# ClashLuke/LocAtE

Measured on AMD Instinct MI355X. Metric: images/sec (G+D step) 64x64 bs=64, higher is better.
Workload: dtype f32 (contractions fp32-faithful on the matrix cores: 2 x scaled fp16 operand pieces / 3 MFMAs per slice where the operand's largest magnitude comes with it, else 3 x bf16 pieces / 6 MFMAs; fp32 accumulate); 1 GPU; LocAtE G+D step, 64x64 RGB, batch 64 per GPU (the fp32 variant - the reference's own precision - of BASELINE.json configs[1]: 64x64 RGB bs 64), self/feature attention at 16x16 and 64x64, random-init weights; global_batch=64, image_size=64, parallelism=dp1, launch=hipGraph replay, G-step generator pass on a second stream

## Files before the change

### locate_amd/csrc/conv.hip

```cpp
#include "igemm.h"



struct PackBatch {
    PackArgs ph[4];
};

__device__ __forceinline__ void pack_tables(const PackArgs& a, int k) {
    int* koff = reinterpret_cast<int*>(a.out + (size_t)a.rows * a.ld);
    unsigned char* ktap = reinterpret_cast<unsigned char*>(koff + a.rows);
    const int T = a.TH * a.TW;
    int off = 0, tap = 31;
    if (k < a.K && T > 0) {
        const int c = k / T, t = k - c * T;
        const int th = t / a.TW, tw = t - th * a.TW;
        off = 4 * (c * a.gHW + (a.dy0 + a.dys * th) * a.gW + a.dx0 + a.dxs * tw - a.dmin);
        tap = t;
    }
    koff[k] = off;
    ktap[k] = (unsigned char)tap;
}

__device__ __forceinline__ void pack_publish_absmax(float m, const PackArgs* phases, int nphase, float* red) {
    m = wave_max(m);
// ... 504 lines not shown
    int nsteps = total_steps - step0;
    if (nsteps > per_split) nsteps = per_split;
    if (nsteps < 0) nsteps = 0;

    const float4* aptr[A_PT];
    bool a_ok[A_PT];
    int a_row[A_PT], a_c4[A_PT];
#pragma unroll
    for (int i = 0; i < A_PT; ++i) {
        const int idx = tid + i * 256;
        const int idc = ((i + 1) * 256 <= A_F4 || idx < A_F4) ? idx : 0;
        a_row[i] = idc / (BM / 4);
        a_c4[i] = idc - a_row[i] * (BM / 4);
        const int col = m0 + a_c4[i] * 4;
        a_ok[i] = col < ph.ld;
        aptr[i] = reinterpret_cast<const float4*>(ph.wp + (long long)(step0 * BK + a_row[i]) * ph.ld + (a_ok[i] ? col : 0));
    }
    const long long a_step = (long long)BK * ph.ld / 4;
    int kidx = step0 * BK + kgrp * KPT;

    float breg[KPT];
    float4 areg[A_PT];
    auto issue_loads = [&]() {
#pragma unroll
        for (int i = 0; i < A_PT; ++i) {
            areg[i] = *aptr[i];
            aptr[i] += a_step;
        }
        const int ks = __builtin_amdgcn_readfirstlane(kidx);
        const i32x8 offs = *reinterpret_cast<const i32x8*>(ph.koff + ks);
        const unsigned long long taps = *reinterpret_cast<const unsigned long long*>(ph.ktap + ks);
#pragma unroll
        for (int j = 0; j < KPT; ++j) breg[j] = gather_load(gc, offs[j], (unsigned)(taps >> (8 * j)) & 31u);
        kidx += BK;
    };
    auto store_tiles = [&](int buf) {
#pragma unroll
        for (int i = 0; i < A_PT; ++i) {
            const int idx = tid + i * 256;
            if ((i + 1) * 256 <= A_F4 || idx < A_F4) {
                float4 v = areg[i];
                v.x = a_ok[i] ? v.x : 0.f; v.y = a_ok[i] ? v.y : 0.f; v.z = a_ok[i] ? v.z : 0.f; v.w = a_ok[i] ? v.w : 0.f;
                *reinterpret_cast<float4*>(&As[buf][a_row[i]][a_c4[i] * 4]) = v;
            }
        }
#pragma unroll
        for (int j = 0; j < KPT; ++j) Bs[buf][kgrp * KPT + j][ncol] = breg[j];
    };

    if (nsteps > 0) {
        issue_loads();
        store_tiles(0);
    }
    __syncthreads();
    const int lrow = lane >> 5, lcol = lane & 31;
    for (int s = 0; s < nsteps; ++s) {
        const int buf = s & 1;
        issue_loads();
        __builtin_amdgcn_sched_barrier(0);
#pragma unroll
        for (int k2 = 0; k2 < BK / 2; ++k2) {
            float a[TM], b[TN];
#pragma unroll
            for (int i = 0; i < TM; ++i) a[i] = As[buf][k2 * 2 + lrow][(wm * TM + i) * 32 + lcol];
#pragma unroll
            for (int j = 0; j < TN; ++j) b[j] = Bs[buf][k2 * 2 + lrow][(wn * TN + j) * 32 + lcol];
#pragma unroll
            for (int i = 0; i < TM; ++i)
#pragma unroll
                for (int j = 0; j < TN; ++j) acc[i][j] = __builtin_amdgcn_mfma_f32_32x32x2f32(a[i], b[j], acc[i][j], 0, 0, 0);
        }
        __builtin_amdgcn_sched_barrier(0);
        store_tiles(buf ^ 1);
        __syncthreads();
    }

    igemm_epilogue<WGM, WGN, TM, TN>(p, ph, acc, col_scale, N, n0, m0, zsplit, wm, wn, lane, nullptr, p.ksplit > 1);
}

#define B6_BK 16

#define IG_FOUR_BLOCKS_TILES 3
#define IG_FOUR_BLOCKS_MIN 2
template <int WGM, int WGN, int TM, int TN, int NP, int NW = 4>
__global__ void __launch_bounds__(64 * NW, (NW == 8 ? 1 : (WGM * TM > 4 ? 2 : ((WGM * TM * TN <= IG_FOUR_BLOCKS_TILES && WGM * TM * TN >= IG_FOUR_BLOCKS_MIN && NP <= 2) ? 4 : 3)))) conv_igemm_bx6_kernel(const IgParams p) {
    constexpr int BK = 4 * NW, KB = BK / 8, KS = BK / 16, NT = 64 * NW;
    constexpr int BM = WGM * TM * 32;
    constexpr int BN = WGN * TN * 32;
    static_assert(NW == 4 || NW == 8, "four or eight waves");
    static_assert(WGM * WGN == NW, "wave grid");
    static_assert(BN == 128 && KB * BN == NT, "one gathered fragment (k-block) per thread and stage");
    static_assert(KB * BM <= 2 * NT, "at most two weight fragments per thread and stage");
    static_assert(B6_BK == 16, "the host's split-K accounting counts 16-deep steps");
    constexpr bool A2 = KB * BM > NT;
    static_assert(2 * BK <= IG_TAIL && (IG_TAIL % 8) == 0, "panel tail shorter than the prefetch distance");

    constexpr int A_U4 = 2 * NP * KB * BM, B_U4 = 2 * NP * KB * BN;
    constexpr int EPI_U4 = (NW * 32 * 33 + 8 + 3) / 4;
    constexpr int SMEM_U4 = A_U4 + B_U4 > EPI_U4 ? A_U4 + B_U4 : EPI_U4;
    __shared__ uint4 smem[SMEM_U4];
    uint4 (*As)[NP][KB][BM] = reinterpret_cast<uint4 (*)[NP][KB][BM]>(smem);
    uint4 (*Bs)[NP][KB][BN] = reinterpret_cast<uint4 (*)[NP][KB][BN]>(smem + A_U4);

    int bx, by, bz;
    xcd_tile(bx, by, bz, p.tile_nphase);
    const int zphase = bz / p.ksplit, zsplit = bz - zphase * p.ksplit;
    const IgPhase& ph = p.ph[zphase];
    const int N = p.B * ph.QH * ph.QW;
    const int n0 = bx * BN;
    const int m0 = by * BM;
    if (n0 >= N) return;

    const int tid = threadIdx.x, lane = tid & 63, wid = tid >> 6;
    const int wm = wid / WGN, wn = wid % WGN;

    const int ncol = tid % BN;
    const int kgrp = __builtin_amdgcn_readfirstlane(tid / BN);
    const GatherCol gc = gather_setup(p, ph, n0 + ncol, N);
    float col_scale[TN];
    igemm_col_scales<WGM, WGN, TM, TN>(p, ph, col_scale, N, n0, wn, lane);
    float b_scale = 1.0f, a_unscale = 1.0f, b_unscale = 1.0f;
    if constexpr (NP == 2) {
        const int kb_ = f16_scale_exp(absmax_read(p.b_absmax));
        const int ka_ = f16_scale_exp(__builtin_amdgcn_readfirstlane(*ph.a_absmax));
        b_scale = pow2f(kb_);
        a_unscale = pow2f(-ka_);
        b_unscale = pow2f(-kb_);
    }

    f32x16 acc[TM][TN];
#pragma unroll
    for (int i = 0; i < TM; ++i)
#pragma unroll
        for (int j = 0; j < TN; ++j)
#pragma unroll
            for (int r = 0; r < 16; ++r) acc[i][j][r] = 0.0f;

    const int total_steps = ph.Kpad / BK;
    const int per_split = (total_steps + p.ksplit - 1) / p.ksplit;
    const int step0 = zsplit * per_split;
    int nsteps = total_steps - step0;
    if (nsteps > per_split) nsteps = per_split;
    if (nsteps < 0) nsteps = 0;

    const bool a_thread = KB * BM == NT || tid < KB * BM;
    const int a_kb = a_thread ? tid / BM : 0, a_m = a_thread ? tid % BM : 0;
    const uint4* ap = ph.w3 + (long long)(step0 * KB + a_kb) * ph.ld + (m0 + a_m);
    const long long a_step = (long long)KB * ph.ld, a_plane = ph.w3_plane;
    const bool b_thread = A2 && tid + NT < KB * BM;
    const int b_kb = b_thread ? (tid + NT) / BM : 0, b_m = b_thread ? (tid + NT) % BM : 0;
    const uint4* bp = ph.w3 + (long long)(step0 * KB + b_kb) * ph.ld + (m0 + b_m);
    int kidx = step0 * BK + kgrp * 8;

    uint4 areg0, areg1, areg2;
    uint4 areg3, areg4, areg5;
    float breg[8];
    i32x8 offs = *reinterpret_cast<const i32x8*>(ph.koff + __builtin_amdgcn_readfirstlane(kidx));
    unsigned long long taps = *reinterpret_cast<const unsigned long long*>(ph.ktap + __builtin_amdgcn_readfirstlane(kidx));
    auto issue_loads = [&]() {
        areg0 = ap[0];
        if constexpr (NP >= 2) areg1 = ap[a_plane];
        if constexpr (NP == 3) areg2 = ap[2 * a_plane];
        ap += a_step;
        if constexpr (A2) {
            areg3 = bp[0];
            if constexpr (NP >= 2) areg4 = bp[a_plane];
            if constexpr (NP == 3) areg5 = bp[2 * a_plane];
            bp += a_step;
        }
#pragma unroll
        for (int j = 0; j < 8; ++j) breg[j] = gather_load(gc, offs[j], (unsigned)(taps >> (8 * j)) & 31u);
        kidx += BK;
        const int ks = __builtin_amdgcn_readfirstlane(kidx);
        offs = *reinterpret_cast<const i32x8*>(ph.koff + ks);
        taps = *reinterpret_cast<const unsigned long long*>(ph.ktap + ks);
    };
    auto store_tiles = [&](int buf) {
        if (a_thread) {
            As[buf][0][a_kb][a_m] = areg0;
            if constexpr (NP >= 2) As[buf][NP >= 2 ? 1 : 0][a_kb][a_m] = areg1;
            if constexpr (NP == 3) As[buf][NP - 1][a_kb][a_m] = areg2;
        }
        if constexpr (A2) {
            if (b_thread) {
                As[buf][0][b_kb][b_m] = areg3;
                if constexpr (NP >= 2) As[buf][NP >= 2 ? 1 : 0][b_kb][b_m] = areg4;
                if constexpr (NP == 3) As[buf][NP - 1][b_kb][b_m] = areg5;
            }
        }
        if constexpr (NP == 2) {
            uint4 h, l;
            float v[8];
#pragma unroll
            for (int j = 0; j < 8; ++j) v[j] = breg[j];
            split2_f16x8(v, b_scale, h, l);
            Bs[buf][0][kgrp][ncol] = h;
            Bs[buf][NP - 1][kgrp][ncol] = l;
        } else if constexpr (NP == 3) {
            uint4 h, m, l;
            float v[8];
#pragma unroll
            for (int j = 0; j < 8; ++j) v[j] = breg[j];
            split3_trunc_x8(v, h, m, l);
            Bs[buf][0][kgrp][ncol] = h;
            Bs[buf][NP - 2][kgrp][ncol] = m;
            Bs[buf][NP - 1][kgrp][ncol] = l;
        } else {
            bf16x8 h;
#pragma unroll
            for (int j = 0; j < 8; ++j) h[j] = (__bf16)breg[j];
            Bs[buf][0][kgrp][ncol] = *reinterpret_cast<uint4*>(&h);
        }
    };

    if (nsteps > 0) {
        issue_loads();
        store_tiles(0);
        issue_loads();
    }
    __syncthreads();
    const int lrow = lane >> 5, lcol = lane & 31;
    constexpr int PROD = NP == 3 ? 6 : (NP == 2 ? 3 : 1);
    constexpr int NMF = TM * TN * PROD, HALF = KS == 1 ? NMF / 2 : NMF;
    using frag_t = typename std::conditional<NP == 2, f16x8, bf16x8>::type;
    for (int s = 0; s < nsteps; ++s) {
        const int buf = s & 1;
        frag_t a[TM][NP], b[TN][NP];
        auto fragments = [&](int ksub) {
#pragma unroll
            for (int i = 0; i < TM; ++i)
#pragma unroll
                for (int q = 0; q < NP; ++q) a[i][q] = *reinterpret_cast<const frag_t*>(&As[buf][q][2 * ksub + lrow][(wm * TM + i) * 32 + lcol]);
#pragma unroll
            for (int j = 0; j < TN; ++j)
#pragma unroll
                for (int q = 0; q < NP; ++q) b[j][q] = *reinterpret_cast<const frag_t*>(&Bs[buf][q][2 * ksub + lrow][(wn * TN + j) * 32 + lcol]);
        };
        fragments(0);
        auto mfmas = [&](int lo, int hi) {
#pragma unroll
            for (int i = 0; i < TM; ++i)
#pragma unroll
                for (int j = 0; j < TN; ++j) {
                    const int base = (i * TN + j) * PROD;
                    if constexpr (NP == 2) {
                        if (base + 0 >= lo && base + 0 < hi) acc[i][j] = __builtin_amdgcn_mfma_f32_32x32x16_f16(a[i][1], b[j][0], acc[i][j], 0, 0, 0);
                        if (base + 1 >= lo && base + 1 < hi) acc[i][j] = __builtin_amdgcn_mfma_f32_32x32x16_f16(a[i][0], b[j][1], acc[i][j], 0, 0, 0);
                        if (base + 2 >= lo && base + 2 < hi) acc[i][j] = __builtin_amdgcn_mfma_f32_32x32x16_f16(a[i][0], b[j][0], acc[i][j], 0, 0, 0);
                    } else if constexpr (NP == 3) {
                        if (base + 0 >= lo && base + 0 < hi) acc[i][j] = __builtin_amdgcn_mfma_f32_32x32x16_bf16(a[i][NP - 1], b[j][0], acc[i][j], 0, 0, 0);
                        if (base + 1 >= lo && base + 1 < hi) acc[i][j] = __builtin_amdgcn_mfma_f32_32x32x16_bf16(a[i][0], b[j][NP - 1], acc[i][j], 0, 0, 0);
                        if (base + 2 >= lo && base + 2 < hi) acc[i][j] = __builtin_amdgcn_mfma_f32_32x32x16_bf16(a[i][NP - 2], b[j][NP - 2], acc[i][j], 0, 0, 0);
                        if (base + 3 >= lo && base + 3 < hi) acc[i][j] = __builtin_amdgcn_mfma_f32_32x32x16_bf16(a[i][NP - 2], b[j][0], acc[i][j], 0, 0, 0);
                        if (base + 4 >= lo && base + 4 < hi) acc[i][j] = __builtin_amdgcn_mfma_f32_32x32x16_bf16(a[i][0], b[j][NP - 2], acc[i][j], 0, 0, 0);
                        if (base + 5 >= lo && base + 5 < hi) acc[i][j] = __builtin_amdgcn_mfma_f32_32x32x16_bf16(a[i][0], b[j][0], acc[i][j], 0, 0, 0);
                    } else {
                        if (base >= lo && base < hi) acc[i][j] = __builtin_amdgcn_mfma_f32_32x32x16_bf16(a[i][0], b[j][0], acc[i][j], 0, 0, 0);
                    }
                }
        };
        __builtin_amdgcn_sched_barrier(0);
        mfmas(0, HALF);
        __builtin_amdgcn_sched_barrier(0);
        store_tiles(buf ^ 1);
        __builtin_amdgcn_sched_barrier(0);
        issue_loads();
        if constexpr (KS == 1) {
            mfmas(HALF, NMF);
        } else {
            fragments(1);
            mfmas(0, NMF);
        }
        if constexpr (NP >= 2) {
#pragma unroll
            for (int k = 0; k < (KS == 1 ? NMF - HALF : NMF); ++k) {
                __builtin_amdgcn_sched_group_barrier(0x008, 1, 0);
                __builtin_amdgcn_sched_group_barrier(0x020, 1, 0);
                __builtin_amdgcn_sched_group_barrier(0x002, 3, 0);
            }
        }
        __syncthreads();
    }
    if constexpr (NP == 2) {
#pragma unroll
        for (int i = 0; i < TM; ++i)
#pragma unroll
            for (int j = 0; j < TN; ++j)
#pragma unroll
                for (int r = 0; r < 16; ++r) acc[i][j][r] = (acc[i][j][r] * a_unscale) * b_unscale;
    }
    float* const stage = reinterpret_cast<float*>(smem) + wid * (32 * 33);
    bool combined = false;
    if (p.ksplit > 1 && p.combine) {
        constexpr int FR = TM * TN * 4;
        const int tile = (zphase * (int)gridDim.y + by) * (int)gridDim.x + bx;
        const int ntiles = p.nphase * (int)gridDim.y * (int)gridDim.x;
        const unsigned tile_bytes = FR * NT * 16;
        __amdgpu_buffer_rsrc_t srs = __builtin_amdgcn_make_buffer_rsrc(p.slab, 0, (int)((unsigned)p.ksplit * ntiles * tile_bytes), 0x00020000);
        const unsigned my = ((unsigned)(zsplit * ntiles + tile)) * tile_bytes + (unsigned)tid * 16u;
#pragma unroll
        for (int i = 0; i < TM; ++i)
#pragma unroll
            for (int j = 0; j < TN; ++j)
#pragma unroll
                for (int q = 0; q < 4; ++q) {
                    u32x4 v;
                    v[0] = __float_as_uint(acc[i][j][4 * q + 0]); v[1] = __float_as_uint(acc[i][j][4 * q + 1]);
                    v[2] = __float_as_uint(acc[i][j][4 * q + 2]); v[3] = __float_as_uint(acc[i][j][4 * q + 3]);
                    __builtin_amdgcn_raw_buffer_store_b128(v, srs, (int)(my + (unsigned)(((i * TN + j) * 4 + q) * NT * 16)), 0, 16);
                }
        asm volatile("s_waitcnt vmcnt(0)" ::: "memory");
        __syncthreads();
        unsigned* const flag = reinterpret_cast<unsigned*>(smem) + NW * 32 * 33 + 4;
        if (tid == 0) {
            const unsigned ticket = __hip_atomic_fetch_add(p.counters + tile, 1u, __ATOMIC_RELAXED, __HIP_MEMORY_SCOPE_AGENT);
            const bool last = ticket == (unsigned)(p.ksplit - 1);
            if (last) {
                __hip_atomic_store(p.counters + tile, 0u, __ATOMIC_RELAXED, __HIP_MEMORY_SCOPE_AGENT);
                __builtin_amdgcn_fence(__ATOMIC_ACQUIRE, "agent");
                asm volatile("s_waitcnt vmcnt(0)" ::: "memory");
            }
            *flag = last ? 1u : 0u;
        }
        __syncthreads();
        if (*flag == 0u) return;
        const unsigned t0 = (unsigned)tile * tile_bytes + (unsigned)tid * 16u;
        const unsigned zstride = (unsigned)ntiles * tile_bytes;
#pragma unroll
        for (int i = 0; i < TM; ++i)
#pragma unroll
            for (int j = 0; j < TN; ++j)
#pragma unroll
                for (int r = 0; r < 16; ++r) acc[i][j][r] = 0.0f;
        constexpr int HB = 4, ZB = 4;
#pragma unroll
        for (int h0 = 0; h0 < FR; h0 += HB) {
            for (int z0 = 0; z0 < p.ksplit; z0 += ZB) {
                u32x4 v[ZB][HB];
#pragma unroll
                for (int zz = 0; zz < ZB; ++zz)
#pragma unroll
                    for (int f = 0; f < HB; ++f)
                        v[zz][f] = __builtin_amdgcn_raw_buffer_load_b128(srs, (int)(t0 + (unsigned)(z0 + zz) * zstride + (unsigned)((h0 + f) * NT * 16)), 0, 16);
#pragma unroll
                for (int zz = 0; zz < ZB; ++zz)
#pragma unroll
                    for (int f = 0; f < HB; ++f) {
                        const int g = h0 + f, i = g / (TN * 4), j = (g / 4) % TN, q = g % 4;
#pragma unroll
                        for (int e = 0; e < 4; ++e) acc[i][j][4 * q + e] += __uint_as_float(v[zz][f][e]);
                    }
            }
        }
        __syncthreads();
        combined = true;
    }
    igemm_epilogue<WGM, WGN, TM, TN>(p, ph, acc, col_scale, N, n0, m0, combined ? 0 : zsplit, wm, wn, lane, stage, p.ksplit > 1 && !combined);
}

__global__ void __launch_bounds__(256) igemm_slab_reduce_kernel(const float* __restrict__ slab, float* __restrict__ out,
                                                                const float* __restrict__ bias, const float* __restrict__ scale,
                                                                int scale_bg, int scale_stride, int B, int M, int plane,
                                                                long long out_bs, long long slab_stride, int ksplit,
// ... 220 lines not shown
template <int PX>
static void launch_pointwise_px(const IgParams& p, hipStream_t st) {
    const long long npx = (long long)p.B * p.H * p.W / PX;
    const int blocks = (int)((npx + 255) / 256);
    const int mt = (p.M + 15) / 16;
    if (mt == 1) conv_pointwise_kernel<16, PX><<<blocks, 256, 0, st>>>(p);
    else if (mt == 2) conv_pointwise_kernel<32, PX><<<blocks, 256, 0, st>>>(p);
    else if (mt == 3) conv_pointwise_kernel<48, PX><<<blocks, 256, 0, st>>>(p);
    else conv_pointwise_kernel<64, PX><<<blocks, 256, 0, st>>>(p);
}

static void launch_pointwise(const IgParams& p, hipStream_t st) {
    if ((long long)p.B * p.H * p.W >= (long long)knob_int("LOCATE_PX2_MIN", 2 * 256 * 1024)) launch_pointwise_px<2>(p, st);
    else launch_pointwise_px<1>(p, st);
}

static int pick_bm(int M);
static int igemm_bm(int M, int nmax, int nphase) {
    if (M % 192 == 0 && M >= 192 && !path_disabled("tall") && !path_disabled("bx6")) {
        const long long tiles = (long long)((nmax + 127) / 128) * (M / 192) * nphase;
        if (tiles >= 512) return 192;
    }
    return pick_bm(M);
}

static int pick_bm(int M) {
    const int cands[4] = {128, 96, 64, 32};
    int best = 128, best_pad = 1 << 30;
    for (int i = 0; i < 4; ++i) {
        const int pad = round_up(M, cands[i]);
        if (pad < best_pad) { best_pad = pad; best = cands[i]; }
    }
    return best;
}

static int igemm_ksplit(int M, int nmax, int nphase, int min_kpad) {
    const int bm = igemm_bm(M, nmax, nphase);
    const long long tiles = (long long)((nmax + 127) / 128) * ((M + bm - 1) / bm) * nphase;
    const int slots = bm == 192 ? 512 : 768;
    if (tiles >= slots || (tiles >= 512 && tiles % 256 == 0)) return 1;
    const int steps = min_kpad / IG_BK;
    long long want = (slots + tiles - 1) / tiles;
    const int min_steps = (long long)M * nmax <= (1 << 16) ? 2 : 8;
    if (steps < 8) return 1;
    const int max_split = steps / min_steps > 0 ? steps / min_steps : 1;
    if (want > max_split) want = max_split;
    if (want > 64) want = 64;
    if (want > knob_int("LOCATE_KS_MAX", 64)) want = knob_int("LOCATE_KS_MAX", 64);
    return want < 1 ? 1 : (int)want;
}

#define IG_MAX_COUNTERS 1024
struct SplitPlan {
    int ksplit, combine, gx, gy;
    size_t slab_floats;
};

static SplitPlan igemm_split_plan(const IgParams& p, int nmax, bool have_counters) {
    SplitPlan sp;
    const int bm = igemm_bm(p.M, nmax, p.nphase);
    int min_kpad = 1 << 30;
    for (int i = 0; i < p.nphase; ++i) min_kpad = p.ph[i].Kpad < min_kpad ? p.ph[i].Kpad : min_kpad;
    int ks = igemm_ksplit(p.M, nmax, p.nphase, min_kpad);
    if (ks > min_kpad / IG_BK) ks = min_kpad / IG_BK;
    if (ks < 1) ks = 1;
    sp.ksplit = ks;
    sp.gx = (nmax + 127) / 128;
    sp.gy = (p.M + bm - 1) / bm;
    const long long ntiles = (long long)sp.gx * sp.gy * p.nphase;
    const long long tile_floats = (long long)bm * 128;
    const long long legacy = ks > 1 ? (long long)ks * p.B * p.M * p.OH * p.OW : 0;
    const long long fused = ks > 1 ? (long long)ks * ntiles * tile_floats : 0;
    sp.combine = have_counters && ks > 1 && (long long)ks * tile_floats * 4 <= (512 << 10) && ntiles <= IG_MAX_COUNTERS &&
                 fused * 4 < (1ll << 31) && (p.precision == 1 || !path_disabled("bx6")) && !path_disabled("combine");
    sp.slab_floats = (size_t)(sp.combine ? fused : legacy);
    return sp;
}

void launch_slab_reduce(const IgParams& p, hipStream_t st) {
    igemm_slab_reduce_kernel<<<stream_grid(p.slab_stride, 256), 256, 0, st>>>(p.slab, p.out, p.bias, p.scale, p.scale_bg, p.scale_stride, p.B, p.M, p.OH * p.OW,
                                                                              p.out_bs, p.slab_stride, p.ksplit, p.act_out, p.act_bs, p.mul_pre, p.mul_bs, p.out_absmax);
}

static int launch_igemm(IgParams& p, int nmax, void* slab_ws, unsigned* counters, hipStream_t st, const char* who) {
    p.tile_nphase = (path_disabled("phasefast") || (long long)p.OH * p.OW < 1024) ? 1 : p.nphase;
    if (p.win) return launch_win_igemm(p, nmax, slab_ws, counters, st, who);
    if (skinny_ok(p)) {
        p.ksplit = 1;
        launch_skinny(p, st);
        LOCATE_LAUNCH_CHECK(who);
        return LOCATE_OK;
    }
    if (pointwise_ok(p)) {
        p.ksplit = 1;
        launch_pointwise(p, st);
        LOCATE_LAUNCH_CHECK(who);
        return LOCATE_OK;
    }
    const int bm = igemm_bm(p.M, nmax, p.nphase);
    const SplitPlan sp = igemm_split_plan(p, nmax, counters != nullptr);
    p.ksplit = sp.ksplit;
    p.combine = sp.combine;
    p.counters = counters;
    p.slab = static_cast<float*>(slab_ws);
    p.slab_stride = (long long)p.B * p.M * p.OH * p.OW;
    dim3 grid(sp.gx, sp.gy, p.nphase * p.ksplit);
    for (int i = 0; i < p.nphase; ++i)
        LOCATE_REQUIRE(round_up(p.M, bm) <= p.ph[i].ld, "%s: tile height %d does not divide the panel width %d", who, bm, p.ph[i].ld);
    if (p.precision == 3) {
        launch_fp8_igemm(p, grid, bm, st);
        LOCATE_LAUNCH_CHECK(who);
        if (p.ksplit > 1 && !p.combine) {
            LOCATE_REQUIRE(p.slab_stride < (1ll << 31), "%s: split-K output of %lld elements exceeds the 32-bit index range", who, p.slab_stride);
            launch_slab_reduce(p, st);
            LOCATE_LAUNCH_CHECK(who);
        }
        return LOCATE_OK;
    }
    const bool w8 = !path_disabled("w8") && !path_disabled("bx6") && (bm == 128 || bm == 64) &&
                    (long long)grid.x * grid.y * grid.z <= knob_int("LOCATE_W8_MAX", 320);
    if (p.precision == 2) LOCATE_REQUIRE(!path_disabled("bx6"), "%s: fp16 pieces need the bf16/fp16 MFMA kernels", who);
    if (w8) {
        if (p.precision == 1) {
            if (bm == 128) conv_igemm_bx6_kernel<2, 4, 2, 1, 1, 8><<<grid, 512, 0, st>>>(p);
            else conv_igemm_bx6_kernel<2, 4, 1, 1, 1, 8><<<grid, 512, 0, st>>>(p);
        } else if (p.precision == 2) {
            if (bm == 128) conv_igemm_bx6_kernel<2, 4, 2, 1, 2, 8><<<grid, 512, 0, st>>>(p);
            else conv_igemm_bx6_kernel<2, 4, 1, 1, 2, 8><<<grid, 512, 0, st>>>(p);
        } else {
            if (bm == 128) conv_igemm_bx6_kernel<2, 4, 2, 1, 3, 8><<<grid, 512, 0, st>>>(p);
            else conv_igemm_bx6_kernel<2, 4, 1, 1, 3, 8><<<grid, 512, 0, st>>>(p);
        }
    } else if (p.precision == 1) {
        if (bm == 192) conv_igemm_bx6_kernel<2, 2, 3, 2, 1><<<grid, 256, 0, st>>>(p);
        else if (bm == 128) conv_igemm_bx6_kernel<2, 2, 2, 2, 1><<<grid, 256, 0, st>>>(p);
        else if (bm == 96) conv_igemm_bx6_kernel<1, 4, 3, 1, 1><<<grid, 256, 0, st>>>(p);
        else if (bm == 64) conv_igemm_bx6_kernel<1, 4, 2, 1, 1><<<grid, 256, 0, st>>>(p);
        else conv_igemm_bx6_kernel<1, 4, 1, 1, 1><<<grid, 256, 0, st>>>(p);
    } else if (p.precision == 2) {
        if (bm == 192) conv_igemm_bx6_kernel<2, 2, 3, 2, 2><<<grid, 256, 0, st>>>(p);
        else if (bm == 128) conv_igemm_bx6_kernel<2, 2, 2, 2, 2><<<grid, 256, 0, st>>>(p);
        else if (bm == 96) conv_igemm_bx6_kernel<1, 4, 3, 1, 2><<<grid, 256, 0, st>>>(p);
        else if (bm == 64) conv_igemm_bx6_kernel<1, 4, 2, 1, 2><<<grid, 256, 0, st>>>(p);
        else conv_igemm_bx6_kernel<1, 4, 1, 1, 2><<<grid, 256, 0, st>>>(p);
    } else if (!path_disabled("bx6")) {
        if (bm == 192) conv_igemm_bx6_kernel<2, 2, 3, 2, 3><<<grid, 256, 0, st>>>(p);
        else if (bm == 128) conv_igemm_bx6_kernel<2, 2, 2, 2, 3><<<grid, 256, 0, st>>>(p);
        else if (bm == 96) conv_igemm_bx6_kernel<1, 4, 3, 1, 3><<<grid, 256, 0, st>>>(p);
        else if (bm == 64) conv_igemm_bx6_kernel<1, 4, 2, 1, 3><<<grid, 256, 0, st>>>(p);
        else conv_igemm_bx6_kernel<1, 4, 1, 1, 3><<<grid, 256, 0, st>>>(p);
    } else {
        if (bm == 128) conv_igemm_kernel<2, 2, 2, 2><<<grid, 256, 0, st>>>(p);
        else if (bm == 96) conv_igemm_kernel<1, 4, 3, 1><<<grid, 256, 0, st>>>(p);
        else if (bm == 64) conv_igemm_kernel<1, 4, 2, 1><<<grid, 256, 0, st>>>(p);
        else conv_igemm_kernel<1, 4, 1, 1><<<grid, 256, 0, st>>>(p);
    }
    LOCATE_LAUNCH_CHECK(who);
    if (p.ksplit > 1 && !p.combine) {
        const long long total = p.slab_stride;
        LOCATE_REQUIRE(total < (1ll << 31), "%s: split-K output of %lld elements exceeds the 32-bit index range", who, total);
        launch_slab_reduce(p, st);
        LOCATE_LAUNCH_CHECK(who);
    }
    return LOCATE_OK;
}

static int launch_pack(const PackBatch& b, int nphase, hipStream_t st, const char* who) {
    const PackJob j = make_pack_job(b, nphase);
    if (b.ph[0].fmt) pack_clear_kernel<<<1, 64, 0, st>>>(j);
    if (b.ph[0].win) {
        if (b.ph[0].fmt) win_absmax_kernel<<<WIN_ABSMAX_BLOCKS, 256, 0, st>>>(j);
        pack_job_kernel<<<j.gx * j.gy, 256, 0, st>>>(j);
        LOCATE_LAUNCH_CHECK(who);
        return LOCATE_OK;
    }
    pack_job_kernel<<<j.gx * j.gy, 256, 0, st>>>(j);
    LOCATE_LAUNCH_CHECK(who);
    int64_t big = 1;
    for (int i = 0; i < nphase; ++i) {
        const int64_t t = (int64_t)(b.ph[i].rows / 8) * b.ph[i].ld;
        if (t > big) big = t;
    }
    pack_split_kernel<<<dim3(stream_grid(big, 256), nphase), 256, 0, st>>>(j);
    LOCATE_LAUNCH_CHECK(who);
    return LOCATE_OK;
}

static ConvGeom make_geom(const int* g) {
    ConvGeom c;
    c.B = g[0]; c.C = g[1]; c.H = g[2]; c.W = g[3]; c.M = g[4]; c.KH = g[5]; c.KW = g[6];
    c.stride = g[7]; c.pad_h = g[8]; c.pad_w = g[9]; c.OH = g[10]; c.OW = g[11];
    return c;
}

static size_t slab_floats(const IgParams& p, int nmax) {
    if (p.win) return win_slab_floats(p, nmax);
    if (skinny_ok(p)) return 0;
    const size_t a = igemm_split_plan(p, nmax, false).slab_floats, b = igemm_split_plan(p, nmax, true).slab_floats;
    return a > b ? a : b;
}

static void useful_taps(int in, int out, int k, int s, int pad, int* lo, int* n) {
    if (path_disabled("taps")) { *lo = 0; *n = k; return; }
    int first = -1, last = -1;
    for (int t = 0; t < k; ++t) {
        bool any = false;
        for (int o = 0; o < out && !any; ++o) {
            const int i = o * s - pad + t;
            any = i >= 0 && i < in;
        }
        if (any) { if (first < 0) first = t; last = t; }
    }
    if (first < 0) { first = 0; last = 0; }
    *lo = first; *n = last - first + 1;
}
static void useful_phase_taps(int Q, int out, int d0, int T, int* lo, int* n) {
    if (path_disabled("taps")) { *lo = 0; *n = T > 0 ? T : 1; return; }
    int first = T > 0 ? d0 - out + 1 : 0, last = d0 + Q - 1;
    if (first < 0) first = 0;
    if (last > T - 1) last = T - 1;
    if (first > last) { first = 0; last = 0; }
    *lo = first; *n = last - first + 1;
}

static void phase_taps(int parity, int pad, int K, int s, int* k0, int* d0, int* T) {
    *k0 = (parity + pad) % s;
    *d0 = (parity + pad - *k0) / s;
    *T = *k0 < K ? (K - *k0 + s - 1) / s : 0;
}

static int tap_dmin(const PackArgs& a) {
    int best = 0;
    for (int th = 0; th < a.TH; ++th)
// ... 1842 lines not shown
```

Before: 7105 images/sec.

## Stream igemm weight tiles into LDS via direct global-to-LDS loads in a ring

The bx6 implicit-GEMM kernel now copies weight tiles straight from global memory into LDS with global_load_lds_dwordx4, skipping the register staging step. It uses a 2- or 3-slot ring buffer, with depth chosen from an LDS budget at compile time, and explicit vmcnt waits. Gathered activations stay double-buffered through registers, the main loop is unrolled by two with alternating gather buffers, and koff/ktap loads go through the constant address space. The aim is to cut VGPR pressure and VALU store work while deepening the prefetch. The cost is inline asm that manipulates m0, fragile hand-counted waitcnt values, and more LDS, which can lower occupancy.

```diff
diff --git a/locate_amd/csrc/conv.hip b/locate_amd/csrc/conv.hip
--- a/locate_amd/csrc/conv.hip
+++ b/locate_amd/csrc/conv.hip
@@ -610,8 +610,14 @@
 
 #define IG_FOUR_BLOCKS_TILES 3
 #define IG_FOUR_BLOCKS_MIN 2
-template <int WGM, int WGN, int TM, int TN, int NP, int NW = 4>
-__global__ void __launch_bounds__(64 * NW, (NW == 8 ? 1 : (WGM * TM > 4 ? 2 : ((WGM * TM * TN <= IG_FOUR_BLOCKS_TILES && WGM * TM * TN >= IG_FOUR_BLOCKS_MIN && NP <= 2) ? 4 : 3)))) conv_igemm_bx6_kernel(const IgParams p) {
+constexpr int bx6_blocks_per_cu(int WGM, int TM, int TN, int NP, int NW) {
+    return NW == 8 ? 1 : (WGM * TM > 4 ? 2 : ((WGM * TM * TN <= IG_FOUR_BLOCKS_TILES && WGM * TM * TN >= IG_FOUR_BLOCKS_MIN && NP <= 2) ? 4 : 3));
+}
+constexpr int bx6_ring_depth(int WGM, int WGN, int TM, int TN, int NP, int NW) {
+    return (3 * WGM * TM * 32 + 2 * WGN * TN * 32) * NP * (NW / 2) * 16 * bx6_blocks_per_cu(WGM, TM, TN, NP, NW) <= 160 * 1024 ? 3 : 2;
+}
+template <int WGM, int WGN, int TM, int TN, int NP, int NW = 4, bool RING = true>
+__global__ void __launch_bounds__(64 * NW, bx6_blocks_per_cu(WGM, TM, TN, NP, NW)) conv_igemm_bx6_kernel(const IgParams p) {
     constexpr int BK = 4 * NW, KB = BK / 8, KS = BK / 16, NT = 64 * NW;
     constexpr int BM = WGM * TM * 32;
     constexpr int BN = WGN * TN * 32;
@@ -621,9 +627,10 @@
     static_assert(KB * BM <= 2 * NT, "at most two weight fragments per thread and stage");
     static_assert(B6_BK == 16, "the host's split-K accounting counts 16-deep steps");
     constexpr bool A2 = KB * BM > NT;
-    static_assert(2 * BK <= IG_TAIL && (IG_TAIL % 8) == 0, "panel tail shorter than the prefetch distance");
-
-    constexpr int A_U4 = 2 * NP * KB * BM, B_U4 = 2 * NP * KB * BN;
+    static_assert(3 * BK <= IG_TAIL && (IG_TAIL % 8) == 0, "panel tail shorter than the prefetch distance");
+    constexpr int RD = RING ? bx6_ring_depth(WGM, WGN, TM, TN, NP, NW) : 2;
+
+    constexpr int A_U4 = RD * NP * KB * BM, B_U4 = 2 * NP * KB * BN;
     constexpr int EPI_U4 = (NW * 32 * 33 + 8 + 3) / 4;
     constexpr int SMEM_U4 = A_U4 + B_U4 > EPI_U4 ? A_U4 + B_U4 : EPI_U4;
     __shared__ uint4 smem[SMEM_U4];
@@ -673,54 +680,27 @@
 
     const bool a_thread = KB * BM == NT || tid < KB * BM;
     const int a_kb = a_thread ? tid / BM : 0, a_m = a_thread ? tid % BM : 0;
-    const uint4* ap = ph.w3 + (long long)(step0 * KB + a_kb) * ph.ld + (m0 + a_m);
     const long long a_step = (long long)KB * ph.ld, a_plane = ph.w3_plane;
     const bool b_thread = A2 && tid + NT < KB * BM;
     const int b_kb = b_thread ? (tid + NT) / BM : 0, b_m = b_thread ? (tid + NT) % BM : 0;
-    const uint4* bp = ph.w3 + (long long)(step0 * KB + b_kb) * ph.ld + (m0 + b_m);
     int kidx = step0 * BK + kgrp * 8;
 
-    uint4 areg0, areg1, areg2;
-    uint4 areg3, areg4, areg5;
-    float breg[8];
     i32x8 offs = *reinterpret_cast<const i32x8*>(ph.koff + __builtin_amdgcn_readfirstlane(kidx));
     unsigned long long taps = *reinterpret_cast<const unsigned long long*>(ph.ktap + __builtin_amdgcn_readfirstlane(kidx));
-    auto issue_loads = [&]() {
-        areg0 = ap[0];
-        if constexpr (NP >= 2) areg1 = ap[a_plane];
-        if constexpr (NP == 3) areg2 = ap[2 * a_plane];
-        ap += a_step;
-        if constexpr (A2) {
-            areg3 = bp[0];
-            if constexpr (NP >= 2) areg4 = bp[a_plane];
-            if constexpr (NP == 3) areg5 = bp[2 * a_plane];
-            bp += a_step;
-        }
-#pragma unroll
-        for (int j = 0; j < 8; ++j) breg[j] = gather_load(gc, offs[j], (unsigned)(taps >> (8 * j)) & 31u);
+    auto gather = [&](float (&g)[8]) {
+#pragma unroll
+        for (int j = 0; j < 8; ++j) g[j] = gather_load(gc, offs[j], (unsigned)(taps >> (8 * j)) & 31u);
         kidx += BK;
         const int ks = __builtin_amdgcn_readfirstlane(kidx);
-        offs = *reinterpret_cast<const i32x8*>(ph.koff + ks);
-        taps = *reinterpret_cast<const unsigned long long*>(ph.ktap + ks);
+        offs = *(const __attribute__((address_space(4))) i32x8*)(ph.koff + ks);
+        taps = *(const __attribute__((address_space(4))) unsigned long long*)(ph.ktap + ks);
     };
-    auto store_tiles = [&](int buf) {
-        if (a_thread) {
-            As[buf][0][a_kb][a_m] = areg0;
-            if constexpr (NP >= 2) As[buf][NP >= 2 ? 1 : 0][a_kb][a_m] = areg1;
-            if constexpr (NP == 3) As[buf][NP - 1][a_kb][a_m] = areg2;
-        }
-        if constexpr (A2) {
-            if (b_thread) {
-                As[buf][0][b_kb][b_m] = areg3;
-                if constexpr (NP >= 2) As[buf][NP >= 2 ? 1 : 0][b_kb][b_m] = areg4;
-                if constexpr (NP == 3) As[buf][NP - 1][b_kb][b_m] = areg5;
-            }
-        }
+    auto store_b = [&](const float (&g)[8], int buf) {
         if constexpr (NP == 2) {
             uint4 h, l;
             float v[8];
 #pragma unroll
-            for (int j = 0; j < 8; ++j) v[j] = breg[j];
+            for (int j = 0; j < 8; ++j) v[j] = g[j];
             split2_f16x8(v, b_scale, h, l);
             Bs[buf][0][kgrp][ncol] = h;
             Bs[buf][NP - 1][kgrp][ncol] = l;
@@ -728,7 +708,7 @@
             uint4 h, m, l;
             float v[8];
 #pragma unroll
-            for (int j = 0; j < 8; ++j) v[j] = breg[j];
+            for (int j = 0; j < 8; ++j) v[j] = g[j];
             split3_trunc_x8(v, h, m, l);
             Bs[buf][0][kgrp][ncol] = h;
             Bs[buf][NP - 2][kgrp][ncol] = m;
@@ -736,69 +716,49 @@
         } else {
             bf16x8 h;
 #pragma unroll
-            for (int j = 0; j < 8; ++j) h[j] = (__bf16)breg[j];
+            for (int j = 0; j < 8; ++j) h[j] = (__bf16)g[j];
             Bs[buf][0][kgrp][ncol] = *reinterpret_cast<uint4*>(&h);
         }
     };
 
-    if (nsteps > 0) {
-        issue_loads();
-        store_tiles(0);
-        issue_loads();
-    }
-    __syncthreads();
     const int lrow = lane >> 5, lcol = lane & 31;
     constexpr int PROD = NP == 3 ? 6 : (NP == 2 ? 3 : 1);
     constexpr int NMF = TM * TN * PROD, HALF = KS == 1 ? NMF / 2 : NMF;
     using frag_t = typename std::conditional<NP == 2, f16x8, bf16x8>::type;
-    for (int s = 0; s < nsteps; ++s) {
-        const int buf = s & 1;
-        frag_t a[TM][NP], b[TN][NP];
-        auto fragments = [&](int ksub) {
-#pragma unroll
-            for (int i = 0; i < TM; ++i)
-#pragma unroll
-                for (int q = 0; q < NP; ++q) a[i][q] = *reinterpret_cast<const frag_t*>(&As[buf][q][2 * ksub + lrow][(wm * TM + i) * 32 + lcol]);
-#pragma unroll
-            for (int j = 0; j < TN; ++j)
-#pragma unroll
-                for (int q = 0; q < NP; ++q) b[j][q] = *reinterpret_cast<const frag_t*>(&Bs[buf][q][2 * ksub + lrow][(wn * TN + j) * 32 + lcol]);
-        };
-        fragments(0);
-        auto mfmas = [&](int lo, int hi) {
-#pragma unroll
-            for (int i = 0; i < TM; ++i)
-#pragma unroll
-                for (int j = 0; j < TN; ++j) {
-                    const int base = (i * TN + j) * PROD;
-                    if constexpr (NP == 2) {
-                        if (base + 0 >= lo && base + 0 < hi) acc[i][j] = __builtin_amdgcn_mfma_f32_32x32x16_f16(a[i][1], b[j][0], acc[i][j], 0, 0, 0);
-                        if (base + 1 >= lo && base + 1 < hi) acc[i][j] = __builtin_amdgcn_mfma_f32_32x32x16_f16(a[i][0], b[j][1], acc[i][j], 0, 0, 0);
-                        if (base + 2 >= lo && base + 2 < hi) acc[i][j] = __builtin_amdgcn_mfma_f32_32x32x16_f16(a[i][0], b[j][0], acc[i][j], 0, 0, 0);
-                    } else if constexpr (NP == 3) {
-                        if (base + 0 >= lo && base + 0 < hi) acc[i][j] = __builtin_amdgcn_mfma_f32_32x32x16_bf16(a[i][NP - 1], b[j][0], acc[i][j], 0, 0, 0);
-                        if (base + 1 >= lo && base + 1 < hi) acc[i][j] = __builtin_amdgcn_mfma_f32_32x32x16_bf16(a[i][0], b[j][NP - 1], acc[i][j], 0, 0, 0);
-                        if (base + 2 >= lo && base + 2 < hi) acc[i][j] = __builtin_amdgcn_mfma_f32_32x32x16_bf16(a[i][NP - 2], b[j][NP - 2], acc[i][j], 0, 0, 0);
-                        if (base + 3 >= lo && base + 3 < hi) acc[i][j] = __builtin_amdgcn_mfma_f32_32x32x16_bf16(a[i][NP - 2], b[j][0], acc[i][j], 0, 0, 0);
-                        if (base + 4 >= lo && base + 4 < hi) acc[i][j] = __builtin_amdgcn_mfma_f32_32x32x16_bf16(a[i][0], b[j][NP - 2], acc[i][j], 0, 0, 0);
-                        if (base + 5 >= lo && base + 5 < hi) acc[i][j] = __builtin_amdgcn_mfma_f32_32x32x16_bf16(a[i][0], b[j][0], acc[i][j], 0, 0, 0);
-                    } else {
-                        if (base >= lo && base < hi) acc[i][j] = __builtin_amdgcn_mfma_f32_32x32x16_bf16(a[i][0], b[j][0], acc[i][j], 0, 0, 0);
-                    }
+    frag_t a[TM][NP], b[TN][NP];
+    auto fragments = [&](int abuf, int bbuf, int ksub) {
+#pragma unroll
+        for (int i = 0; i < TM; ++i)
+#pragma unroll
+            for (int q = 0; q < NP; ++q) a[i][q] = *reinterpret_cast<const frag_t*>(&As[abuf][q][2 * ksub + lrow][(wm * TM + i) * 32 + lcol]);
+#pragma unroll
+        for (int j = 0; j < TN; ++j)
+#pragma unroll
+            for (int q = 0; q < NP; ++q) b[j][q] = *reinterpret_cast<const frag_t*>(&Bs[bbuf][q][2 * ksub + lrow][(wn * TN + j) * 32 + lcol]);
+    };
+    auto mfmas = [&](int lo, int hi) {
+#pragma unroll
+        for (int i = 0; i < TM; ++i)
+#pragma unroll
+            for (int j = 0; j < TN; ++j) {
+                const int base = (i * TN + j) * PROD;
+                if constexpr (NP == 2) {
+                    if (base + 0 >= lo && base + 0 < hi) acc[i][j] = __builtin_amdgcn_mfma_f32_32x32x16_f16(a[i][1], b[j][0], acc[i][j], 0, 0, 0);
+                    if (base + 1 >= lo && base + 1 < hi) acc[i][j] = __builtin_amdgcn_mfma_f32_32x32x16_f16(a[i][0], b[j][1], acc[i][j], 0, 0, 0);
+                    if (base + 2 >= lo && base + 2 < hi) acc[i][j] = __builtin_amdgcn_mfma_f32_32x32x16_f16(a[i][0], b[j][0], acc[i][j], 0, 0, 0);
+                } else if constexpr (NP == 3) {
+                    if (base + 0 >= lo && base + 0 < hi) acc[i][j] = __builtin_amdgcn_mfma_f32_32x32x16_bf16(a[i][NP - 1], b[j][0], acc[i][j], 0, 0, 0);
+                    if (base + 1 >= lo && base + 1 < hi) acc[i][j] = __builtin_amdgcn_mfma_f32_32x32x16_bf16(a[i][0], b[j][NP - 1], acc[i][j], 0, 0, 0);
+                    if (base + 2 >= lo && base + 2 < hi) acc[i][j] = __builtin_amdgcn_mfma_f32_32x32x16_bf16(a[i][NP - 2], b[j][NP - 2], acc[i][j], 0, 0, 0);
+                    if (base + 3 >= lo && base + 3 < hi) acc[i][j] = __builtin_amdgcn_mfma_f32_32x32x16_bf16(a[i][NP - 2], b[j][0], acc[i][j], 0, 0, 0);
+                    if (base + 4 >= lo && base + 4 < hi) acc[i][j] = __builtin_amdgcn_mfma_f32_32x32x16_bf16(a[i][0], b[j][NP - 2], acc[i][j], 0, 0, 0);
+                    if (base + 5 >= lo && base + 5 < hi) acc[i][j] = __builtin_amdgcn_mfma_f32_32x32x16_bf16(a[i][0], b[j][0], acc[i][j], 0, 0, 0);
+                } else {
+                    if (base >= lo && base < hi) acc[i][j] = __builtin_amdgcn_mfma_f32_32x32x16_bf16(a[i][0], b[j][0], acc[i][j], 0, 0, 0);
                 }
-        };
-        __builtin_amdgcn_sched_barrier(0);
-        mfmas(0, HALF);
-        __builtin_amdgcn_sched_barrier(0);
-        store_tiles(buf ^ 1);
-        __builtin_amdgcn_sched_barrier(0);
-        issue_loads();
-        if constexpr (KS == 1) {
-            mfmas(HALF, NMF);
-        } else {
-            fragments(1);
-            mfmas(0, NMF);
-        }
+            }
+    };
+    auto interleave = [&]() {
         if constexpr (NP >= 2) {
 #pragma unroll
             for (int k = 0; k < (KS == 1 ? NMF - HALF : NMF); ++k) {
@@ -807,6 +767,150 @@
                 __builtin_amdgcn_sched_group_barrier(0x002, 3, 0);
             }
         }
+    };
+
+    if constexpr (!RING) {
+        const uint4* ap = ph.w3 + (long long)(step0 * KB + a_kb) * ph.ld + (m0 + a_m);
+        const uint4* bp = ph.w3 + (long long)(step0 * KB + b_kb) * ph.ld + (m0 + b_m);
+        uint4 areg0, areg1, areg2;
+        uint4 areg3, areg4, areg5;
+        float breg[8];
+        auto issue_loads = [&]() {
+            areg0 = ap[0];
+            if constexpr (NP >= 2) areg1 = ap[a_plane];
+            if constexpr (NP == 3) areg2 = ap[2 * a_plane];
+            ap += a_step;
+            if constexpr (A2) {
+                areg3 = bp[0];
+                if constexpr (NP >= 2) areg4 = bp[a_plane];
+                if constexpr (NP == 3) areg5 = bp[2 * a_plane];
+                bp += a_step;
+            }
+            gather(breg);
+        };
+        auto store_tiles = [&](int buf) {
+            if (a_thread) {
+                As[buf][0][a_kb][a_m] = areg0;
+                if constexpr (NP >= 2) As[buf][NP >= 2 ? 1 : 0][a_kb][a_m] = areg1;
+                if constexpr (NP == 3) As[buf][NP - 1][a_kb][a_m] = areg2;
+            }
+            if constexpr (A2) {
+                if (b_thread) {
+                    As[buf][0][b_kb][b_m] = areg3;
+                    if constexpr (NP >= 2) As[buf][NP >= 2 ? 1 : 0][b_kb][b_m] = areg4;
+                    if constexpr (NP == 3) As[buf][NP - 1][b_kb][b_m] = areg5;
+                }
+            }
+            store_b(breg, buf);
+        };
+
+        if (nsteps > 0) {
+            issue_loads();
+            store_tiles(0);
+            issue_loads();
+        }
+        __syncthreads();
+        for (int s = 0; s < nsteps; ++s) {
+            const int buf = s & 1;
+            fragments(buf, buf, 0);
+            __builtin_amdgcn_sched_barrier(0);
+            mfmas(0, HALF);
+            __builtin_amdgcn_sched_barrier(0);
+            store_tiles(buf ^ 1);
+            __builtin_amdgcn_sched_barrier(0);
+            issue_loads();
+            if constexpr (KS == 1) {
+                mfmas(HALF, NMF);
+            } else {
+                fragments(buf, buf, 1);
+                mfmas(0, NMF);
+            }
+            interleave();
+            __syncthreads();
+        }
+    } else {
+        constexpr int A_WAVES = (KB * BM < NT ? KB * BM : NT) / 64, B_WAVES = A2 ? (KB * BM - NT) / 64 : 0;
+        static_assert((KB * BM) % 64 == 0, "whole waves copy the weight chunks");
+        const int wv = __builtin_amdgcn_readfirstlane(wid);
+        const bool a_wave = wv < A_WAVES, b_wave = A2 && wv < B_WAVES;
+        const unsigned lds0 = (unsigned)reinterpret_cast<uintptr_t>(smem);
+        unsigned a_off = (unsigned)(((long long)(step0 * KB + a_kb) * ph.ld + (m0 + a_m)) * 16);
+        unsigned b_off = (unsigned)(((long long)(step0 * KB + b_kb) * ph.ld + (m0 + b_m)) * 16);
+        const unsigned off_step = (unsigned)(a_step * 16);
+        auto copy16 = [&](unsigned lds_dst, const uint4* plane, unsigned voff) {
+            unsigned keep;
+            asm volatile("s_mov_b32 %0, m0\n\ts_mov_b32 m0, %1\n\ts_nop 0\n\tglobal_load_lds_dwordx4 %2, %3\n\ts_mov_b32 m0, %0"
+                         : "=&s"(keep) : "s"(lds_dst), "v"(voff), "s"(plane) : "memory");
+        };
+        auto copy_weights = [&](int slot) {
+            if (a_wave) {
+#pragma unroll
+                for (int q = 0; q < NP; ++q) copy16(lds0 + (unsigned)(((slot * NP + q) * KB * BM + wv * 64) * 16), ph.w3 + q * a_plane, a_off);
+            }
+            if constexpr (A2) {
+                if (b_wave) {
+#pragma unroll
+                    for (int q = 0; q < NP; ++q) copy16(lds0 + (unsigned)(((slot * NP + q) * KB * BM + NT + wv * 64) * 16), ph.w3 + q * a_plane, b_off);
+                }
+                b_off += off_step;
+            }
+            a_off += off_step;
+        };
+        auto wait_weights = [&]() {
+            if constexpr (RD == 2) {
+                if (a_wave) asm volatile("s_waitcnt vmcnt(8)" ::: "memory");
+            } else {
+                if (b_wave) asm volatile("s_waitcnt vmcnt(%0)" :: "i"(16 + 2 * NP) : "memory");
+                else if (a_wave) asm volatile("s_waitcnt vmcnt(%0)" :: "i"(16 + NP) : "memory");
+            }
+        };
+        float g0[8], g1[8];
+        auto stage = [&](int s, int slot, float (&g)[8]) {
+            const int bbuf = s & 1;
+            fragments(slot, bbuf, 0);
+            __builtin_amdgcn_sched_barrier(0);
+            mfmas(0, HALF);
+            __builtin_amdgcn_sched_barrier(0);
+            store_b(g, bbuf ^ 1);
+            __builtin_amdgcn_sched_barrier(0);
+            copy_weights(slot == 0 ? RD - 1 : slot - 1);
+            __builtin_amdgcn_sched_barrier(0);
+            gather(g);
+            if constexpr (KS == 1) {
+                mfmas(HALF, NMF);
+            } else {
+                fragments(slot, bbuf, 1);
+                mfmas(0, NMF);
+            }
+            interleave();
+            __builtin_amdgcn_sched_barrier(0);
+            wait_weights();
+            __syncthreads();
+        };
+        if (nsteps > 0) {
+            gather(g0);
+            if constexpr (RD == 3) {
+                copy_weights(0);
+                gather(g1);
+                copy_weights(1);
+            } else {
+                gather(g1);
+                copy_weights(0);
+            }
+            store_b(g0, 0);
+            gather(g0);
+            wait_weights();
+        }
+        __syncthreads();
+        int s = 0, slot = 0;
+        for (; s + 2 <= nsteps; s += 2) {
+            stage(s, slot, g1);
+            slot = slot == RD - 1 ? 0 : slot + 1;
+            stage(s + 1, slot, g0);
+            slot = slot == RD - 1 ? 0 : slot + 1;
+        }
+        if (s < nsteps) stage(s, slot, g1);
+        asm volatile("s_waitcnt vmcnt(0)" ::: "memory");
         __syncthreads();
     }
     if constexpr (NP == 2) {
@@ -1193,6 +1297,40 @@
                                                                               p.out_bs, p.slab_stride, p.ksplit, p.act_out, p.act_bs, p.mul_pre, p.mul_bs, p.out_absmax);
 }
 
+template <bool RING>
+static void launch_bx6(const IgParams& p, dim3 grid, int bm, bool w8, hipStream_t st) {
+    if (w8) {
+        if (p.precision == 1) {
+            if (bm == 128) conv_igemm_bx6_kernel<2, 4, 2, 1, 1, 8, RING><<<grid, 512, 0, st>>>(p);
+            else conv_igemm_bx6_kernel<2, 4, 1, 1, 1, 8, RING><<<grid, 512, 0, st>>>(p);
+        } else if (p.precision == 2) {
+            if (bm == 128) conv_igemm_bx6_kernel<2, 4, 2, 1, 2, 8, RING><<<grid, 512, 0, st>>>(p);
+            else conv_igemm_bx6_kernel<2, 4, 1, 1, 2, 8, RING><<<grid, 512, 0, st>>>(p);
+        } else {
+            if (bm == 128) conv_igemm_bx6_kernel<2, 4, 2, 1, 3, 8, RING><<<grid, 512, 0, st>>>(p);
+            else conv_igemm_bx6_kernel<2, 4, 1, 1, 3, 8, RING><<<grid, 512, 0, st>>>(p);
+        }
+    } else if (p.precision == 1) {
+        if (bm == 192) conv_igemm_bx6_kernel<2, 2, 3, 2, 1, 4, RING><<<grid, 256, 0, st>>>(p);
+        else if (bm == 128) conv_igemm_bx6_kernel<2, 2, 2, 2, 1, 4, RING><<<grid, 256, 0, st>>>(p);
+        else if (bm == 96) conv_igemm_bx6_kernel<1, 4, 3, 1, 1, 4, RING><<<grid, 256, 0, st>>>(p);
+        else if (bm == 64) conv_igemm_bx6_kernel<1, 4, 2, 1, 1, 4, RING><<<grid, 256, 0, st>>>(p);
+        else conv_igemm_bx6_kernel<1, 4, 1, 1, 1, 4, RING><<<grid, 256, 0, st>>>(p);
+    } else if (p.precision == 2) {
+        if (bm == 192) conv_igemm_bx6_kernel<2, 2, 3, 2, 2, 4, RING><<<grid, 256, 0, st>>>(p);
+        else if (bm == 128) conv_igemm_bx6_kernel<2, 2, 2, 2, 2, 4, RING><<<grid, 256, 0, st>>>(p);
+        else if (bm == 96) conv_igemm_bx6_kernel<1, 4, 3, 1, 2, 4, RING><<<grid, 256, 0, st>>>(p);
+        else if (bm == 64) conv_igemm_bx6_kernel<1, 4, 2, 1, 2, 4, RING><<<grid, 256, 0, st>>>(p);
+        else conv_igemm_bx6_kernel<1, 4, 1, 1, 2, 4, RING><<<grid, 256, 0, st>>>(p);
+    } else {
+        if (bm == 192) conv_igemm_bx6_kernel<2, 2, 3, 2, 3, 4, RING><<<grid, 256, 0, st>>>(p);
+        else if (bm == 128) conv_igemm_bx6_kernel<2, 2, 2, 2, 3, 4, RING><<<grid, 256, 0, st>>>(p);
+        else if (bm == 96) conv_igemm_bx6_kernel<1, 4, 3, 1, 3, 4, RING><<<grid, 256, 0, st>>>(p);
+        else if (bm == 64) conv_igemm_bx6_kernel<1, 4, 2, 1, 3, 4, RING><<<grid, 256, 0, st>>>(p);
+        else conv_igemm_bx6_kernel<1, 4, 1, 1, 3, 4, RING><<<grid, 256, 0, st>>>(p);
+    }
+}
+
 static int launch_igemm(IgParams& p, int nmax, void* slab_ws, unsigned* counters, hipStream_t st, const char* who) {
     p.tile_nphase = (path_disabled("phasefast") || (long long)p.OH * p.OW < 1024) ? 1 : p.nphase;
     if (p.win) return launch_win_igemm(p, nmax, slab_ws, counters, st, who);
@@ -1231,35 +1369,14 @@
     const bool w8 = !path_disabled("w8") && !path_disabled("bx6") && (bm == 128 || bm == 64) &&
                     (long long)grid.x * grid.y * grid.z <= knob_int("LOCATE_W8_MAX", 320);
     if (p.precision == 2) LOCATE_REQUIRE(!path_disabled("bx6"), "%s: fp16 pieces need the bf16/fp16 MFMA kernels", who);
-    if (w8) {
-        if (p.precision == 1) {
-            if (bm == 128) conv_igemm_bx6_kernel<2, 4, 2, 1, 1, 8><<<grid, 512, 0, st>>>(p);
-            else conv_igemm_bx6_kernel<2, 4, 1, 1, 1, 8><<<grid, 512, 0, st>>>(p);
-        } else if (p.precision == 2) {
-            if (bm == 128) conv_igemm_bx6_kernel<2, 4, 2, 1, 2, 8><<<grid, 512, 0, st>>>(p);
-            else conv_igemm_bx6_kernel<2, 4, 1, 1, 2, 8><<<grid, 512, 0, st>>>(p);
-        } else {
-            if (bm == 128) conv_igemm_bx6_kernel<2, 4, 2, 1, 3, 8><<<grid, 512, 0, st>>>(p);
-            else conv_igemm_bx6_kernel<2, 4, 1, 1, 3, 8><<<grid, 512, 0, st>>>(p);
-        }
-    } else if (p.precision == 1) {
-        if (bm == 192) conv_igemm_bx6_kernel<2, 2, 3, 2, 1><<<grid, 256, 0, st>>>(p);
-        else if (bm == 128) conv_igemm_bx6_kernel<2, 2, 2, 2, 1><<<grid, 256, 0, st>>>(p);
-        else if (bm == 96) conv_igemm_bx6_kernel<1, 4, 3, 1, 1><<<grid, 256, 0, st>>>(p);
-        else if (bm == 64) conv_igemm_bx6_kernel<1, 4, 2, 1, 1><<<grid, 256, 0, st>>>(p);
-        else conv_igemm_bx6_kernel<1, 4, 1, 1, 1><<<grid, 256, 0, st>>>(p);
-    } else if (p.precision == 2) {
-        if (bm == 192) conv_igemm_bx6_kernel<2, 2, 3, 2, 2><<<grid, 256, 0, st>>>(p);
-        else if (bm == 128) conv_igemm_bx6_kernel<2, 2, 2, 2, 2><<<grid, 256, 0, st>>>(p);
-        else if (bm == 96) conv_igemm_bx6_kernel<1, 4, 3, 1, 2><<<grid, 256, 0, st>>>(p);
-        else if (bm == 64) conv_igemm_bx6_kernel<1, 4, 2, 1, 2><<<grid, 256, 0, st>>>(p);
-        else conv_igemm_bx6_kernel<1, 4, 1, 1, 2><<<grid, 256, 0, st>>>(p);
-    } else if (!path_disabled("bx6")) {
-        if (bm == 192) conv_igemm_bx6_kernel<2, 2, 3, 2, 3><<<grid, 256, 0, st>>>(p);
-        else if (bm == 128) conv_igemm_bx6_kernel<2, 2, 2, 2, 3><<<grid, 256, 0, st>>>(p);
-        else if (bm == 96) conv_igemm_bx6_kernel<1, 4, 3, 1, 3><<<grid, 256, 0, st>>>(p);
-        else if (bm == 64) conv_igemm_bx6_kernel<1, 4, 2, 1, 3><<<grid, 256, 0, st>>>(p);
-        else conv_igemm_bx6_kernel<1, 4, 1, 1, 3><<<grid, 256, 0, st>>>(p);
+    if (p.precision != 0 || !path_disabled("bx6")) {
+        for (int i = 0; i < p.nphase; ++i)
+            LOCATE_REQUIRE(p.ph[i].w3_plane < (1ll << 28), "%s: weight panel piece of %lld chunks exceeds 4 GiB", who, p.ph[i].w3_plane);
+#ifdef LOCATE_DEBUG_KNOBS
+        if (path_disabled("ring")) launch_bx6<false>(p, grid, bm, w8, st);
+        else
+#endif
+            launch_bx6<true>(p, grid, bm, w8, st);
     } else {
         if (bm == 128) conv_igemm_kernel<2, 2, 2, 2><<<grid, 256, 0, st>>>(p);
         else if (bm == 96) conv_igemm_kernel<1, 4, 3, 1><<<grid, 256, 0, st>>>(p);
```

New measurement: 7129 images/sec (median of 6 runs). No clear change (+0.3%).
